# yhz0/SQLP

Measured on AMD Instinct MI355X. Metric: stage-2 subproblems/sec + cut-gen HBM GB/s on STORM, higher is better.
Workload: dtype f64

## Files before the change

### include/twosd_hip.h

```cpp
#ifndef TWOSD_HIP_H
#define TWOSD_HIP_H

#include <stdint.h>

#ifdef __cplusplus
extern "C" {
#endif

typedef struct twosd_ctx twosd_ctx;

enum {
    TWOSD_OK = 0,
    TWOSD_E_ARG = -1,
    TWOSD_E_DEVICE = -2,
    TWOSD_E_STATE = -3,
    TWOSD_E_LP = -4,
    TWOSD_E_UNSUPPORTED = -5
};

enum { TWOSD_LP_OPTIMAL = 0, TWOSD_LP_INFEASIBLE = 1, TWOSD_LP_ITER_LIMIT = 2, TWOSD_LP_NUMERIC = 3 };

const char *twosd_last_error(void);

const char *twosd_version(void);
// ... 152 lines not shown
int twosd_bootstrap_count_of_word(uint32_t u);
int twosd_bootstrap_counts(twosd_ctx *ctx, int M, uint64_t seed, uint64_t first_index, int64_t count, uint8_t *out);

int twosd_bootstrap_counts_vr(twosd_ctx *ctx, int M, uint64_t seed, uint64_t first_index, int64_t count, uint8_t *out,
                              const twosd_sampling *plan);

int twosd_reform_cuts(twosd_ctx *ctx, int epi, int H, const int *handles, int M, uint64_t seed, uint64_t index_offset,
                      double *alpha, double *beta, double *weight_mark, double *total_weight);
int twosd_reform_partial_len(twosd_ctx *ctx, int H, const int *handles, int M, int64_t *n_u64, int64_t *n_f64);
int twosd_reform_partial(twosd_ctx *ctx, int epi, int H, const int *handles, int M, uint64_t seed, uint64_t index_offset,
                         double total_weight, uint64_t *d_u64, double *d_f64);
int twosd_reform_finalize(twosd_ctx *ctx, int H, const int *handles, int M, double total_weight, const uint64_t *d_u64,
                          const double *d_f64, double *alpha, double *beta, double *weight_mark, double *total_weight_out);
int twosd_reform_cuts_vr(twosd_ctx *ctx, int epi, int H, const int *handles, int M, uint64_t seed, uint64_t index_offset,
                         double *alpha, double *beta, double *weight_mark, double *total_weight, const twosd_sampling *plan);
int twosd_reform_partial_vr(twosd_ctx *ctx, int epi, int H, const int *handles, int M, uint64_t seed, uint64_t index_offset,
                            double total_weight, uint64_t *d_u64, double *d_f64, const twosd_sampling *plan);
int twosd_reform_last_ms(twosd_ctx *ctx, double *ms2);

int twosd_last_timings(twosd_ctx *ctx, double *us5);

int twosd_last_lp_stats(twosd_ctx *ctx, int64_t *pivots_sum, int *pivots_max);
int twosd_last_lp_eta_entries(twosd_ctx *ctx, int64_t *entries, int64_t *retries);

int twosd_last_objective(twosd_ctx *ctx, double *weighted_sum, double *weight_sum);

int twosd_last_lp_iters(twosd_ctx *ctx, int N, int *iters, int *status);

int twosd_set_refresh_kcap(twosd_ctx *ctx, int kcap);

int twosd_last_lp_ops(twosd_ctx *ctx, int64_t *row_ops, int *row_width);

int twosd_debug_stamps(twosd_ctx *ctx, uint64_t *out10, int reset);

#ifdef __cplusplus
}
#endif
#endif
```

### sqlp_amd/_lib.py

```python
from __future__ import annotations

import ctypes as C
import os

_HERE = os.path.dirname(os.path.abspath(__file__))
LIB_PATH = os.path.join(_HERE, f"libtwosd_hip_{os.environ['TWOSD_LIB']}.so" if os.environ.get("TWOSD_LIB")
                        else "libtwosd_hip.so")

TWOSD_OK = 0
ERRORS = {-1: "TWOSD_E_ARG", -2: "TWOSD_E_DEVICE", -3: "TWOSD_E_STATE", -4: "TWOSD_E_LP",
          -5: "TWOSD_E_UNSUPPORTED"}
LP_OPTIMAL, LP_INFEASIBLE, LP_ITER_LIMIT, LP_NUMERIC = 0, 1, 2, 3

P = C.c_void_p
I = C.c_int
D = C.c_double
SIGNATURES = [
    ("twosd_last_error", C.c_char_p, []),
    ("twosd_version", C.c_char_p, []),
    ("twosd_create", I, [I, P]),
    ("twosd_destroy", I, [P]),
    ("twosd_set_template", I, [P, I, I, I, P, P, P, P, P, P, P, P, P, P, P, I]),
    ("twosd_lp_shape", I, [P, P, P, P]),
    ("twosd_canonical_form", I, [I, I, P, P, P, P, P, P, P, P, I, P, P, P, P, P, P, P, P, P, P, P, P, P, P, P]),
# ... 20 lines not shown
    ("twosd_moments_merge", I, [P, P, P]),
    ("twosd_moments_of_values", I, [P, C.c_int64, P, P, P]),
    ("twosd_evaluate_moments", I, [P, P, C.c_int64, C.c_int64, C.c_uint64, P]),
    ("twosd_evaluate_paired", I, [P, P, P, C.c_int64, C.c_int64, C.c_uint64, P, P, P]),
    ("twosd_evaluate_ci", I, [P, P, C.c_uint64, C.c_int64, C.c_int64, C.c_int64, D, D, D, D, P, P, P]),
    ("twosd_solve_batch", I, [P, I, P, I, I, P, P, P, P]),
    ("twosd_solve_values", I, [P, P, I, P, P, P, P, P]),
    ("twosd_dvs_push", I, [P, I, P, P, P]),
    ("twosd_dvs_size", I, [P, P]),
    ("twosd_dvs_get", I, [P, I, I, P]),
    ("twosd_dvs_clear", I, [P]),
    ("twosd_dvs_truncate", I, [P, I]),
    ("twosd_dvs_fingerprint", I, [P, P]),
    ("twosd_solve_push", I, [P, I, P, I, I, P, P, P]),
    ("twosd_last_push_reps", I, [P, P]),
    ("twosd_last_push_mode", I, [P, P]),
    ("twosd_build_cut", I, [P, I, P, D, P, P, P, P, P]),
    ("twosd_cut_partial_len", I, [P, P, P]),
    ("twosd_cut_partial", I, [P, I, P, D, D, P, P, P, P]),
    ("twosd_cut_finalize", I, [P, P, P, P, P, P]),
    ("twosd_last_timings", I, [P, P]),
    ("twosd_last_lp_stats", I, [P, P, P]),
    ("twosd_last_lp_eta_entries", I, [P, P, P]),
    ("twosd_last_lp_ops", I, [P, P, P]),
    ("twosd_debug_stamps", I, [P, P, I]),
    ("twosd_last_lp_iters", I, [P, I, P, P]),
    ("twosd_set_refresh_kcap", I, [P, I]),
    ("twosd_refresh_train", I, [P, I, P, I, I, P, P, P]),
    ("twosd_refresh_train_ex", I, [P, I, P, I, I, I, P, P, P, P]),
    ("twosd_refresh_cap_stats", I, [P, P, P]),
    ("twosd_training_cap", I, [P, C.c_int64, C.c_int64, P]),
    ("twosd_cut_stats", I, [P, P]),
    ("twosd_cut_pass", I, [P, P, P]),
    ("twosd_cut_pass_kind", I, [P, P, P, P]),
    ("twosd_cut_debug_scores", I, [P, I, P, P, C.c_int64, P, P]),
    ("twosd_select_refresh_bases", I, [P, P, P, P, I, I, P, P, P]),
    ("twosd_last_objective", I, [P, P, P]),
    ("twosd_refresh_train_bases", I, [P, P, P, P]),
    ("twosd_refresh_build_local", I, [P, I, P, P]),
    ("twosd_refresh_pack", I, [P, P]),
    ("twosd_refresh_assemble", I, [P, I, P, C.c_int64, I, P, P, P, P]),
    ("twosd_pool_candidate_picks", I, [P, I, P, I, I, I, P, P]),
    ("twosd_pool_set_candidates", I, [P, I, I, I, P, P]),
    ("twosd_picks_keep", I, [P, I, P]),
    ("twosd_picks_info", I, [P, I, P, P, P]),
    ("twosd_picks_get", I, [P, I, P]),
# ... 65 lines not shown
```

### sqlp_amd/csrc/lp_batch.hip

```cpp
#include <hip/hip_runtime.h>
#include <algorithm>
#include <cmath>
#include <cstdio>
#include <cstdlib>
#include <vector>
#include "twosd_internal.h"
#include "twosd_ctx.h"

using namespace twosd;

int twosd::run_lp(twosd_ctx *c, const double *x, const double *d_dv, int N, const LpRun &o) {
    const bool want_pi = o.want_pi, want_y = o.want_y;
    const bool list = o.d_list != nullptr;
    const int NL = list ? o.nlist : N;
    int rc;
    if ((rc = prepare_x(c, x))) return rc;
    if (list && c->pool.size() > 1 && (size_t)N > c->d_pool_pick.cap) return fail(TWOSD_E_STATE, "LP list mode: no recorded pool picks");
    const int m = c->L.m, n = c->L.n, MP = c->MP, R = c->R;
    if (N > c->out_cap) {
        size_t cap = std::max<size_t>(N, 1024);
        if ((rc = c->d_obj.alloc(cap)) || (rc = c->d_status.alloc(cap)) || (rc = c->d_iters.alloc(cap)) ||
            (rc = c->d_ops.alloc(cap)) || (rc = c->d_etan.alloc(cap)))
            return rc;
        c->d_pi.release(); c->d_y.release();
        c->out_cap = (int)cap;
    }
    if (want_pi && (size_t)NL * m > c->d_pi.cap && (rc = c->d_pi.alloc((size_t)c->out_cap * m))) return rc;
    if (o.want_key && (size_t)N > c->d_vkey.cap && (rc = c->d_vkey.alloc((size_t)c->out_cap))) return rc;
    if (o.want_bkey && (size_t)N > c->d_bkey.cap && (rc = c->d_bkey.alloc((size_t)c->out_cap))) return rc;
    if (want_y && (size_t)N * n > c->d_y.cap && (rc = c->d_y.alloc((size_t)c->out_cap * n))) return rc;
    if (!c->d_queue && (rc = c->d_queue.alloc((size_t)kMaxQueueGroups * kQueueStride))) return rc;
    {
        const int CH = c->CH;
        int kmax = c->kmax_override > 0 ? c->kmax_override : std::min(256, std::max(64, 2 * m + 32));
        if (c->kmax_override <= 0 && 2 * m + 32 > kmax) {
            const int b0 = hyper_max_blocks_per_cu(R, CH, kmax, c->k);
            for (int k2 = std::min(1024, (2 * m + 32) & ~31); k2 > kmax; k2 -= 32)
                if (hyper_max_blocks_per_cu(R, CH, k2, c->k) >= b0) { kmax = k2; break; }
        }
        const int ecap = (int)std::min<long long>(INT32_MAX / 2, (long long)std::max(4096, 32 * MP) * std::max(256, kmax) / 256);
        int bpc = hyper_max_blocks_per_cu(R, CH, kmax, c->k);
        if (const char *e = getenv("TWOSD_BPC")) bpc = std::min(bpc, std::max(1, atoi(e)));
        if (bpc < 1)
            return fail(TWOSD_E_UNSUPPORTED, "LP kernel: LDS slice too large (m2 = %d, n2 = %d; LP: %d rows, %d columns; k = %d)",
                        c->m2_user, c->n2_user, m, n, c->k);
        const int nblocks = std::max(1, std::min((NL + kWavesPerBlock - 1) / kWavesPerBlock, bpc * c->num_cus));
        const size_t slots = (size_t)nblocks * kWavesPerBlock;
        if (slots > c->earena_slots || ecap != c->earena_cap) {
            if ((rc = c->d_eidx.alloc(slots * ecap)) || (rc = c->d_evals.alloc(slots * ecap))) return rc;
            c->earena_slots = slots;
            c->earena_cap = ecap;
        }
        HIPCHK(hipMemsetAsync(c->d_queue, 0, sizeof(int) * kMaxQueueGroups * kQueueStride, c->stream));
        HyperParams H{};
        H.m = m; H.n = n; H.k = c->k; H.N = NL; H.kmax = kmax; H.ecap = ecap;
        H.kcap = o.kcap > 0 ? std::min(o.kcap, kmax) : kmax;
        H.retry = o.kcap > 0 ? 0 : 1;
        H.colptr = c->d_colptr; H.rowidx = c->d_rowidx; H.val = c->d_val; H.q = c->d_q; H.btype = c->d_btype;
        H.wcp = c->d_wcp; H.wcc = c->d_wcc; H.wcv = c->d_wcv;
        H.bcp = c->d_bcp; H.bci = c->d_bci; H.bcv = c->d_bcv;
        H.brptr = c->d_brptr; H.brcol = c->d_brcol; H.brval = c->d_brval;
        H.kslot = c->d_kslot; H.kix = c->d_kix; H.kv = c->d_kv; H.kcoef = c->d_kcoef;
        H.xbase = c->d_xbase; H.d0 = c->d_d0; H.hb0 = c->d_hb0;
        H.basic0 = c->d_basic0; H.fixedmask = c->d_fixedmask; H.ubmask = c->d_ubmask;
        H.dv = d_dv; H.eidx = c->d_eidx; H.evals = c->d_evals; H.queue = c->d_queue;
        H.qgroups = std::max(1, std::min(16, nblocks));
        if (const char *e = getenv("TWOSD_QGROUPS")) H.qgroups = std::max(1, std::min({kMaxQueueGroups, nblocks, atoi(e)}));
        H.obj = c->d_obj; H.pi = want_pi ? c->d_pi : nullptr; H.y = want_y ? c->d_y : nullptr;
        H.vkey = o.want_key ? c->d_vkey : nullptr;
        H.key_zero = 1e-12;
        if (const char *e = getenv("TWOSD_KEY_ZERO")) H.key_zero = atof(e);
        H.bkey = o.want_bkey ? c->d_bkey : nullptr;
        if (o.want_etas) {
            const size_t need = list ? (size_t)NL : (size_t)N;
            if (need * 4096 > (size_t)INT32_MAX)
                return fail(TWOSD_E_UNSUPPORTED, "eta files of %zu solves exceed the 2^31-entry arena (at most %d)", need,
                            INT32_MAX / 4096);
            const size_t cap_need = std::max(std::max<size_t>(need, 256) * 4096, c->eo_min_cap);
// ... 43 lines not shown
                int w = 0;
                for (int t = 0; t < R; ++t) w = std::max(w, ks[(size_t)p * (R + 1) + t + 1] - ks[(size_t)p * (R + 1) + t]);
                ws[p] = w;
                mean += w;
            }
            std::sort(ws.begin(), ws.end());
            fprintf(stderr, "LP start: ELL width w over %d bases: min %d, median %d, mean %.2f, p90 %d, max %d\n", H.npool, ws.front(),
                    ws[ws.size() / 2], mean / H.npool, ws[ws.size() * 9 / 10], ws.back());
        }
        HIPCHK(hipEventRecord(c->ev[EV_LP_BEGIN], c->stream));
        const int *order = nullptr;
        if (list) {
            order = o.d_list;
        } else if (H.npool > 1) {
            if ((rc = select_pool(c, d_dv, N, c->d_pool_pick, 0))) return rc;
            order = c->d_order;
        }
        HIPCHK(hipEventRecord(c->ev[EV_LP_SELECTED], c->stream));
        if (order || H.npool > 1) {
            if ((rc = c->d_qrec.fit(std::max<size_t>(NL, 1024)))) return rc;
            HIPCHK(launch_queue_records(order, H.npool > 1 ? c->d_pool_pick : nullptr, c->d_qrec, NL, c->stream));
            H.qrec = c->d_qrec;
        }
        HIPCHK(launch_hyper(R, CH, H, nblocks, hyper_lds_bytes(R, CH, kmax, c->k), c->stream));
        HIPCHK(hipEventRecord(c->ev[EV_LP_END], c->stream));
        HIPCHK(hipStreamSynchronize(c->stream));
        float ms = 0, ms_sel = 0;
        hipEventElapsedTime(&ms, c->ev[EV_LP_SELECTED], c->ev[EV_LP_END]);
        hipEventElapsedTime(&ms_sel, c->ev[EV_LP_BEGIN], c->ev[EV_LP_SELECTED]);
        if (list) {
            if (o.lp_us_out) *o.lp_us_out = 1e3 * ms;
            return TWOSD_OK;
        }
        c->last.N = N;
        c->last.lp_us = 1e3 * ms;
        c->last.sel_us = 1e3 * ms_sel;
        return TWOSD_OK;
    }
}

__global__ void __launch_bounds__(256) lp_stats_kernel(int N, const int *__restrict__ its, const long long *__restrict__ ops,
                                                      const int *__restrict__ st, const int *__restrict__ etan,
                                                      unsigned long long *out) {
    __shared__ unsigned long long red[4][5];
    unsigned long long a = 0, b = 0, d = 0, e = 0;
    unsigned long long mx = 0;
    for (int s = blockIdx.x * blockDim.x + threadIdx.x; s < N; s += gridDim.x * blockDim.x) {
// ... 184 lines not shown
    us5[T_POOL_SELECT] = c->last.sel_us;
    return TWOSD_OK;
}

extern "C" int twosd_last_lp_eta_entries(twosd_ctx *c, int64_t *entries, int64_t *retries) {
    if (!c || !entries) return fail(TWOSD_E_ARG, "last_lp_eta_entries: NULL");
    *entries = c->last.eta_entries;
    if (retries) *retries = c->last.retries;
    return TWOSD_OK;
}

extern "C" int twosd_last_lp_stats(twosd_ctx *c, int64_t *sum, int *mx) {
    if (!c) return fail(TWOSD_E_ARG, "last_lp_stats: NULL");
    if (sum) *sum = c->last.pivots_sum;
    if (mx) *mx = c->last.pivots_max;
    return TWOSD_OK;
}

extern "C" int twosd_last_lp_iters(twosd_ctx *c, int N, int *iters, int *status) {
    if (!c || N < 0 || N > c->out_cap || !c->d_iters) return fail(TWOSD_E_ARG, "last_lp_iters: N = %d outside the last batch", N);
    HIPCHK(hipStreamSynchronize(c->stream));
    if (iters) HIPCHK(hipMemcpy(iters, c->d_iters, sizeof(int) * N, hipMemcpyDeviceToHost));
    if (status) HIPCHK(hipMemcpy(status, c->d_status, sizeof(int) * N, hipMemcpyDeviceToHost));
    return TWOSD_OK;
}

extern "C" int twosd_debug_stamps(twosd_ctx *c, uint64_t *out10, int reset) {
    if (!c || !out10) return fail(TWOSD_E_ARG, "debug_stamps: NULL");
    for (int i = 0; i < 10; ++i) out10[i] = 0;
    if (!c->d_stamps) return TWOSD_OK;
    HIPCHK(hipMemcpy(out10, c->d_stamps, sizeof(uint64_t) * 10, hipMemcpyDeviceToHost));
    if (reset) HIPCHK(hipMemset(c->d_stamps, 0, sizeof(uint64_t) * 16));
    return TWOSD_OK;
}

extern "C" int twosd_last_lp_ops(twosd_ctx *c, int64_t *row_ops, int *row_width) {
    if (!c) return fail(TWOSD_E_ARG, "last_lp_ops: NULL");
    if (row_ops) *row_ops = c->last.ops_sum;
    if (row_width) *row_width = 1;
    return TWOSD_OK;
}

__global__ void gather_rows_kernel(int U, int m, const int *__restrict__ list, const double *__restrict__ pi, double *__restrict__ out) {
    const size_t tot = (size_t)U * m;
    for (size_t i = (size_t)blockIdx.x * blockDim.x + threadIdx.x; i < tot; i += (size_t)gridDim.x * blockDim.x) {
        const int u = (int)(i / m), r = (int)(i % m);
// ... 98 lines not shown
```

### sqlp_amd/csrc/lp_hyper.hip

```cpp
#include <hip/hip_runtime.h>
#include <math.h>
#include <type_traits>
#include "twosd_internal.h"
#include "wave_ops.h"

namespace twosd {

#define HTOL_P 1e-9
#define HTOL_D 1e-9
#define HTOL_PIV 1e-9
#define HPI_ZERO 1e-12


#ifdef TWOSD_STAMPS
#define STAMP_DECL unsigned long long st_acc[10] = {0, 0, 0, 0, 0, 0, 0, 0, 0, 0}; \
    unsigned long long st_last = __builtin_amdgcn_s_memtime();
#define STAMP(i)                                                      \
    {                                                                 \
        const unsigned long long t_ = __builtin_amdgcn_s_memtime();   \
        st_acc[i] += t_ - st_last;                                    \
        st_last = t_;                                                 \
    }
#define STAMP_FLUSH                                                                         \
    if (lane == 0 && P.stamps)                                                              \
// ... 104 lines not shown
    int v = 0;
    H_SLOT_SWITCH(__builtin_amdgcn_readfirstlane(p >> 6), R, {
        int u = a[SL];
        asm volatile("" : "+v"(u));
        v = __builtin_amdgcn_readlane(u, p & 63);
    })
    return v;
}

__device__ __forceinline__ int h_prefix_count(uint64_t m) {
    return __builtin_amdgcn_mbcnt_hi((unsigned)(m >> 32), __builtin_amdgcn_mbcnt_lo((unsigned)m, 0u));
}

__device__ __forceinline__ const __attribute__((address_space(4))) HyperParams *h_args() {
    uint64_t a = (uint64_t)__builtin_amdgcn_kernarg_segment_ptr();
    asm volatile("" : "+s"(a));
    return (const __attribute__((address_space(4))) HyperParams *)a;
}
#define CP (*h_args())

static __host__ __device__ inline int hyper_union_doubles(int R, int C) {
    return 128 * R > 64 * C ? 128 * R : 64 * C;
}
static __host__ __device__ inline size_t hyper_slice_bytes(int R, int C, int kmax, int k) {
    const int kmaxp = (kmax + 3) & ~3;
    return 8 * (size_t)hyper_union_doubles(R, C) + 8 * (size_t)((k + 1) & ~1) + 8 * 64 + 4 * 64 + 4 * 64 + 2 * kmaxp +
           4 * (kmaxp + 4);
}
size_t hyper_lds_bytes(int R, int C, int kmax, int k) { return (size_t)kWavesPerBlock * hyper_slice_bytes(R, C, kmax, k); }

#ifndef TWOSD_ETA_G
#define TWOSD_ETA_G 2
#endif
constexpr int EG = TWOSD_ETA_G;
#ifndef TWOSD_REC_UNROLL
#define TWOSD_REC_UNROLL 1
#endif
#ifndef TWOSD_XB_U
#define TWOSD_XB_U 1
#endif
constexpr int XU = TWOSD_XB_U;
#ifndef TWOSD_HYPER_WPE
#define TWOSD_HYPER_WPE(R) ((R) >= 9 ? 2 : 3)
#endif

template <int R, int C, bool FULL>
__global__ void __launch_bounds__(256, TWOSD_HYPER_WPE(R)) lp_hyper_kernel(HyperParams P) {
    extern __shared__ double lds_raw[];
    using Mask = typename std::conditional<(C > 32), uint64_t, uint32_t>::type;
    const int lane = threadIdx.x & 63;
    const int wid = threadIdx.x >> 6;
    constexpr int MP = 64 * R;
    constexpr int UD = 128 * R > 64 * C ? 128 * R : 64 * C;
    const int kmaxp = (P.kmax + 3) & ~3;
    const int ncol = P.n + P.m;
    char *slice = reinterpret_cast<char *>(lds_raw) + (size_t)wid * hyper_slice_bytes(R, C, P.kmax, P.k);
    double *ut = reinterpret_cast<double *>(slice);
    double *rho = ut + MP;
    double *alpha = ut;
    double *dvl = ut + UD;
    double *lstv = dvl + ((P.k + 1) & ~1);
    int *lsti = reinterpret_cast<int *>(lstv + 64);
    int *smark = lsti + 64;
    unsigned short *etap = reinterpret_cast<unsigned short *>(smark + 64);
    int *etaoff = reinterpret_cast<int *>(etap + kmaxp);

    const int m = P.m, n = P.n;
    const int slot_id = blockIdx.x * kWavesPerBlock + wid;
    int *eidx = P.eidx + (size_t)slot_id * P.ecap;
    double *evals = P.evals + (size_t)slot_id * P.ecap;
    const uint64_t fixedm = CP.fixedmask[lane];
    const uint64_t ubm = CP.ubmask[lane];

    for (int j = lane; j < UD; j += 64) ut[j] = 0.0;
    smark[lane] = 0;
    h_wave_sync();
    STAMP_DECL

    const int G = CP.qgroups;
    const int g0 = blockIdx.x % G;
    int gt = 0;
    int q_lo = 0, q_hi = 0;
    auto group_of = [&](int gi) { return g0 + gi < G ? g0 + gi : g0 + gi - G; };
    auto range_set = [&]() {
        const int g = group_of(gt);
        q_lo = (int)(((long long)P.N * g) / G);
        q_hi = (int)(((long long)P.N * (g + 1)) / G);
    };
    auto claim_issue = [&]() -> int {
        int t = 0;
        if (lane == 0 && gt < G) t = atomicAdd(CP.queue + group_of(gt) * kQueueStride, 1);
        return t;
    };
// ... 106 lines not shown
#pragma unroll
                for (int uu = 0; uu < XU; ++uu)
#pragma unroll
                    for (int t = 0; t < R; ++t) {
                        const double v = fma(kvv[uu][t], dg[uu][t], xB[t]);
                        xB[t] = u0 + uu < len[t] ? v : xB[t];
                    }
            }
            uint64_t ub = ubm;
            asm volatile("" : "+v"(ub));
#pragma unroll
            for (int c = 0; c < C; ++c) d[c] = h_flip(d0r[c], ((ub >> c) & 1) << 63);
            if (attempt == 0 && q_nx >= 0) {
                s_nx = has_rec ? __builtin_amdgcn_readfirstlane(rcn.x) : q_nx;
                pb_nx = has_rec ? __builtin_amdgcn_readfirstlane(rcn.y) : 0;
            }
        }
        K = 0; status = TWOSD_LP_OPTIMAL; eoff = 0;
        if (lane == 0) etaoff[0] = 0;
        h_wave_sync();
        STAMP(0)

        auto eta_group = [&](int t0, int dir, int (&gi)[EG], double (&gv)[EG], int (&gn)[EG], int (&go)[EG]) {
#pragma unroll
            for (int g = 0; g < EG; ++g) {
                const int tt = t0 + dir * g;
                const bool ok = (tt >= 0) & (tt < K);
                const int tc = ok ? tt : 0;
                const int o0 = etaoff[tc], o1 = etaoff[tc + 1];
                go[g] = ok ? o0 : 0;
                gn[g] = ok ? o1 - o0 : 0;
                const bool mine = lane < gn[g];
                const int at = mine ? go[g] + lane : 0;
                const int ix = eidx[at];
                const double vx = evals[at];
                gi[g] = mine ? ix : 0;
                gv[g] = mine ? vx : 0.0;
            }
        };
        for (;;) {
            double bnum = 0.0, bden = 1.0, bdel = 0.0;
            int br = 0x7fffffff;
#pragma unroll
            for (int t = 0; t < R; ++t) {
                const int bt = hb[t] & 3;
                const bool inf = (hb[t] >= 0) & (((xB[t] < -HTOL_P) & (bt != BT_G)) | ((xB[t] > HTOL_P) & ((bt & 1) != 0)));
                if (__builtin_amdgcn_ballot_w64(inf) != 0 && inf) {
                    const double dl = xB[t];
                    const double num = dl * dl, den = (double)wd[t];
                    if (num * bden > bnum * den) { bnum = num; bden = den; br = 64 * t + lane; bdel = dl; }
                }
            }
            const ArgBest1 lr = warg_max1(bnum / bden, br, bdel);
            const int r = lr.idx;
            STAMP(1)
            if (lr.key == 0.0) break;
            if (K >= P.kcap) { status = TWOSD_LP_ITER_LIMIT; break; }
            const double delta = lr.p0;

            auto price_batch = [&](int nb) {
                h_wave_sync();
                int p0 = 0, len = 0;
// ... 27 lines not shown
                    lstv[pos] = gr;
                }
                nops += rlen;
                if (nzm != 0) price_batch(__popcll(nzm));
            } else {
                {
                    double one = 1.0;
                    asm volatile("" : "+v"(one));
                    if (lane == (r & 63)) ut[r] = one;
                }
                h_wave_sync();
                const int gp0 = lane <= K ? (lane == 0 ? r : (int)etap[K - lane]) : -1;
                int bp0 = 0, bp1 = 0;
                if (gp0 >= 0) {
                    bp0 = brptr[gp0];
                    bp1 = brptr[gp0 + 1];
                }
                {
                    auto apply = [&](int tg, const int (&gi)[EG], const double (&gv)[EG], const int (&gn)[EG], const int (&go)[EG]) {
#pragma unroll
                        for (int g = 0; g < EG; ++g) {
                            const int tt = tg - g;
                            if (tt < 0) break;
                            const double ug = gv[g] != 0.0 ? ut[gi[g]] : 0.0;
                            if (gn[g] <= 64 && __builtin_amdgcn_ballot_w64(ug != 0.0) == 0) {
                                nops += gn[g];
                                continue;
                            }
                            double acc = ug * gv[g];
                            for (int e = 64 + lane; e < gn[g]; e += 64) acc = fma(ut[eidx[go[g] + e]], evals[go[g] + e], acc);
                            acc = wsum(acc);
                            nops += gn[g];
                            if (lane == 0) ut[etap[tt]] = acc;
                            h_wave_sync();
                        }
                    };
                    int ai[EG], an[EG], ao[EG], bi[EG], bn[EG], bo[EG];
                    double av[EG], bv[EG];
                    if (K <= 2 * EG) {
                        for (int tg = K - 1; tg >= 0; tg -= EG) {
                            eta_group(tg, -1, ai, av, an, ao);
                            apply(tg, ai, av, an, ao);
                        }
                    } else {
                        eta_group(K - 1, -1, ai, av, an, ao);
                        for (int tg = K - 1; tg >= 0;) {
                            eta_group(tg - EG, -1, bi, bv, bn, bo);
                            apply(tg, ai, av, an, ao);
                            tg -= EG;
                            if (tg < 0) break;
                            eta_group(tg - EG, -1, ai, av, an, ao);
                            apply(tg, bi, bv, bn, bo);
                            tg -= EG;
// ... 67 lines not shown
                const bool el = (((cand >> c) & 1) != 0) & (a > HTOL_PIV);
                snz = h_uniform(snz | ((Mask)(__builtin_amdgcn_ballot_w64(av != 0.0) != 0) << c));
                if (__builtin_amdgcn_ballot_w64(el) != 0) {
                    sel |= (Mask)1 << c;
                    const double nu = d[c] + HTOL_D;
                    const bool better = el & (nu * bde < bnu * a);
                    bnu = better ? nu : bnu;
                    bde = better ? a : bde;
                    elm |= (Mask)el << c;
                }
                __builtin_amdgcn_sched_barrier(0);
            }
            const double thmax = wmin(bnu / bde);
            if (thmax == INFINITY) {
                status = TWOSD_LP_INFEASIBLE;
                h_wave_sync();
#pragma unroll
                for (int c = 0; c < C; ++c) alpha[64 * c + lane] = 0.0;
                break;
            }
            double bA = 0.0, bD = 0.0;
            int bq = 0x7fffffff;
            apf = alpha[lane];
#pragma unroll
            for (int c = 0; c < C; ++c) {
                const double av = apf;
                if (c + 1 < C) apf = alpha[64 * (c + 1) + lane];
                if ((sel >> c) & 1) {
                    const double a = h_flip(av, sgm);
                    const bool ok = (((elm >> c) & 1) != 0) & (d[c] <= thmax * a) & (a > bA);
                    bA = ok ? a : bA;
                    bD = ok ? d[c] : bD;
                    bq = ok ? 64 * c + lane : bq;
                }
                __builtin_amdgcn_sched_barrier(0);
            }
            const ArgBest1 eq = warg_max1(bA, bq, bD);
            const int q = eq.idx;
            STAMP(5)
            if (eq.key == 0.0) {
                status = TWOSD_LP_NUMERIC;
                h_wave_sync();
#pragma unroll
                for (int c = 0; c < C; ++c) alpha[64 * c + lane] = 0.0;
                break;
            }
            const double thetaD = eq.p0 / eq.key;
            int fq = q;
            asm volatile("" : "+v"(fq));
            const bool fcol = q < n;
            int fn0 = 0, fn1 = 1, fcc = 0, fp0 = 0, fp1 = 0;
            double ffa = 0.0;
            apf = alpha[lane];
#pragma unroll
            for (int c = 0; c < C; ++c) {
                if (c == 0 && fcol) {
// ... 29 lines not shown
                    if (pw < np1) {
                        const int cc = P.rowidx[pw];
                        fa = P.val[pw];
                        p0 = bcp[cc];
                        len = bcp[cc + 1] - p0;
                    }
                    nops += h_seg_scatter(p0, len, fa, P.bci, P.bcv, ut, smark, lane);
                }
            }
            h_wave_sync();
            {
                auto apply = [&](int tg, const int (&gi)[EG], const double (&gv)[EG], const int (&gn)[EG], const int (&go)[EG]) {
#pragma unroll
                    for (int g = 0; g < EG; ++g) {
                        const int tt = tg + g;
                        if (tt >= K) break;
                        const int p = etap[tt];
                        const double vp = ut[p];
                        if (vp != 0.0) {
                            if (lane < gn[g]) {
                                if (gi[g] == p) ut[p] = gv[g] * vp;
                                else lds_add(&ut[gi[g]], gv[g] * vp);
                            }
                            for (int e = 64 + lane; e < gn[g]; e += 64) {
                                const int i = eidx[go[g] + e];
                                const double ev = evals[go[g] + e];
                                if (i == p) ut[p] = ev * vp;
                                else lds_add(&ut[i], ev * vp);
                            }
                            nops += gn[g];
                            h_wave_sync();
                        }
                    }
                };
                int ai[EG], an[EG], ao[EG], bi[EG], bn[EG], bo[EG];
                double av[EG], bv[EG];
                if (K <= 2 * EG) {
                    for (int tg = 0; tg < K; tg += EG) {
                        eta_group(tg, 1, ai, av, an, ao);
                        apply(tg, ai, av, an, ao);
                    }
                } else {
                    eta_group(0, 1, ai, av, an, ao);
                    for (int tg = 0; tg < K;) {
                        eta_group(tg + EG, 1, bi, bv, bn, bo);
                        apply(tg, ai, av, an, ao);
                        tg += EG;
                        if (tg >= K) break;
                        eta_group(tg + EG, 1, ai, av, an, ao);
                        apply(tg, bi, bv, bn, bo);
                        tg += EG;
// ... 3 lines not shown
            const double arq = ut[r];
            double col[R];
#pragma unroll
            for (int t = 0; t < R; ++t) col[t] = ut[64 * t + lane];
            h_wave_sync();
#pragma unroll
            for (int t = 0; t < R; ++t) ut[64 * t + lane] = 0.0;
            STAMP(7)
            if (fabs(arq) < 1e-12) { status = TWOSD_LP_NUMERIC; h_wave_sync(); break; }

            const double thetaP = delta / arq;
            const double inv_arq = 1.0 / arq;
            float wrr = 0.0f;
            H_SLOT_SWITCH(__builtin_amdgcn_readfirstlane(r >> 6), R, {
                int u = __builtin_bit_cast(int, wd[SL]);
                asm volatile("" : "+v"(u));
                wrr = __builtin_bit_cast(float, __builtin_amdgcn_readlane(u, r & 63));
            })
            int cnt = 0;
#pragma unroll
            for (int t = 0; t < R; ++t) cnt += __popcll(__ballot(col[t] != 0.0));
            if (eoff + cnt > P.ecap) { status = TWOSD_LP_ITER_LIMIT; h_wave_sync(); break; }
            int base = eoff;
#pragma unroll
            for (int t = 0; t < R; ++t) {
                const int i = 64 * t + lane;
                const bool nz = col[t] != 0.0;
                const bool isr = i == r;
                const uint64_t bal = __ballot(nz);
                const double ratio = col[t] * inv_arq;
                if (nz) {
                    const int pos = base + h_prefix_count(bal);
                    eidx[pos] = i;
                    evals[pos] = isr ? inv_arq : -ratio;
                }
                const float nw = (float)((double)wrr * inv_arq * inv_arq);
                const float cand = (float)(ratio * ratio * (double)wrr);
                const double xo = fma(-thetaP, col[t], xB[t]);
                xB[t] = isr ? thetaP : (nz ? xo : xB[t]);
                wd[t] = isr ? (nw > 1.0f ? nw : 1.0f) : ((nz & (cand > wd[t])) ? cand : wd[t]);
                base += __popcll(bal);
            }
            eoff += cnt;
            if (lane == 0) {
                etap[K] = (unsigned short)r;
                etaoff[K + 1] = eoff;
            }
            ++K;
            const int lh = h_get_row_i<R>(hb, r);
            const int leaving = lh >> 2;
            {
                const int ls = __builtin_amdgcn_readfirstlane(leaving >> 6), qs = __builtin_amdgcn_readfirstlane(q >> 6);
                const double dlv = (delta > 0) == ((lh & 3) == BT_G) ? thetaD : -thetaD;
                const bool lme = lane == (leaving & 63), qme = lane == (q & 63);
                H_SLOT_SWITCH(ls, C, {
                    double v = lme ? dlv : d[SL];
                    asm volatile("" : "+v"(v));
                    d[SL] = v;
                })
                H_SLOT_SWITCH(qs, C, {
                    double v = qme ? 0.0 : d[SL];
                    asm volatile("" : "+v"(v));
                    d[SL] = v;
                })
                if (lme) bmask &= ~(1ull << ls);
                if (qme) bmask |= 1ull << qs;
                {
                    const int nh = q * 4 + (int)P.btype[q];
                    const bool rme = lane == (r & 63);
                    H_SLOT_SWITCH(__builtin_amdgcn_readfirstlane(r >> 6), R, {
                        int v = rme ? nh : hb[SL];
                        asm volatile("" : "+v"(v));
                        hb[SL] = v;
                    })
                }
            }
            ++it;
            h_wave_sync();
            STAMP(8)
        }
        if (status == TWOSD_LP_OPTIMAL || pb == 0 || !CP.retry) break;
        if (lane == 0 && CP.retries) atomicAdd(CP.retries, 1ull);
        pb = 0;
        }
        double dvn0 = 0.0, dvn1 = 0.0, kcn0 = 0.0, kcn1 = 0.0;
        int ksn = 0, t_claim = 0;
        if (q_nx >= 0) {
            const auto *A = h_args();
            t_claim = claim_issue();
            if (lane <= R) ksn = A->kslot[pb_nx * (R + 1) + lane];
            if (dv_pf) {
                const double *dvs = A->dv + (size_t)s_nx * P.k;
                if (lane < P.k) { dvn0 = dvs[lane]; kcn0 = A->kcoef[lane]; }
                if (lane + 64 < P.k) { dvn1 = dvs[lane + 64]; kcn1 = A->kcoef[lane + 64]; }
            }
        }

        double objv = NAN;
        unsigned long long keyv = 0;
        if (status == TWOSD_LP_OPTIMAL) {
            const double *qc = CP.q;
            double qv[R];
#pragma unroll
// ... 43 lines not shown
                        const double v = fabs(dc) <= zt ? 0.0 : dc;
                        const unsigned long long b = ((unsigned long long)__double_as_longlong(v) + (1ull << 28)) >> 29;
                        h += mix64(((unsigned long long)(j - n) << 35) | b);
                    }
                }
#pragma unroll
                for (int o = 32; o > 0; o >>= 1) h += __shfl_xor(h, o);
                keyv = h;
            }
        }
        if constexpr (FULL) {
        if (status == TWOSD_LP_OPTIMAL && (P.pi || P.y)) {
            const double *qc = CP.q;
#pragma unroll
            for (int t = 0; t < R; ++t) {
                const int j = hb[t] >> 2;
                const bool bq = hb[t] >= 0 && j < n;
                const double qj = qc[bq ? j : 0];
                ut[64 * t + lane] = bq ? qj : 0.0;
            }
            h_wave_sync();
            for (int tt = K - 1; tt >= 0; --tt) {
                const int off = etaoff[tt], nnz = etaoff[tt + 1] - off;
                double acc = 0.0;
                for (int e = lane; e < nnz; e += 64) acc = fma(ut[eidx[off + e]], evals[off + e], acc);
                acc = wsum(acc);
                nops += nnz;
                if (lane == 0) ut[etap[tt]] = acc;
                h_wave_sync();
            }
            double pv[R];
            double pmax = 0.0;
#pragma unroll
            for (int t = 0; t < R; ++t) {
                const int cc = 64 * t + lane;
                const int e0 = cc < m ? bcp[cc] : 0, e1 = cc < m ? bcp[cc + 1] : 0;
                double a = 0.0;
#pragma unroll TWOSD_REC_UNROLL
                for (int e = e0; e < e1; ++e) a = fma(ut[P.bci[e]], P.bcv[e], a);
                pv[t] = a;
                pmax = fmax(pmax, fabs(a));
            }
            nops += P.bnnz[pb];
            pmax = wmax(pmax);
            const double zt = HPI_ZERO * (1.0 + pmax);
#pragma unroll
            for (int t = 0; t < R; ++t)
                if (fabs(pv[t]) <= zt) pv[t] = 0.0;
// ... 26 lines not shown
        if (P.head_out) {
            const size_t ho = (size_t)(P.pi_by_pos ? qpos : s) * m;
#pragma unroll
            for (int t = 0; t < R; ++t)
                if (64 * t + lane < m) P.head_out[ho + 64 * t + lane] = hb[t] >> 2;
        }
        if (P.bkey && status == TWOSD_LP_OPTIMAL) {
            unsigned long long h = 0;
#pragma unroll
            for (int t = 0; t < R; ++t)
                if (64 * t + lane < m) h += mix64((unsigned long long)(hb[t] >> 2));
#pragma unroll
            for (int o = 32; o > 0; o >>= 1) h += __shfl_xor(h, o);
            if (lane == 0) P.bkey[s] = h;
        }
        if (P.eo_K) {
            const int erow = P.pi_by_pos ? qpos : s;
            unsigned long long off64 = 0;
            if (lane == 0 && status == TWOSD_LP_OPTIMAL) off64 = atomicAdd(P.eo_used, (unsigned long long)eoff);
            off64 = __shfl(off64, 0);
            const bool ok = status == TWOSD_LP_OPTIMAL && off64 + (unsigned long long)eoff <= (unsigned long long)P.eo_cap;
            const int off = ok ? (int)off64 : 0;
            if (ok) {
                for (int e = lane; e < eoff; e += 64) {
                    P.eo_eidx[off + e] = eidx[e];
                    P.eo_evals[off + e] = evals[e];
                }
                for (int t = lane; t < K; t += 64) P.eo_etap[(size_t)erow * P.kmax + t] = etap[t];
                for (int t = lane; t <= K; t += 64) P.eo_etaoff[(size_t)erow * (P.kmax + 1) + t] = etaoff[t];
            }
            if (lane == 0) {
                P.eo_K[erow] = ok ? K : -1;
                P.eo_off[erow] = off;
                P.eo_pb[erow] = pb;
            }
        }
        }
        {
            const auto *A = h_args();
            double *const o_obj = A->obj;
            int *const o_status = A->status, *const o_iters = A->iters, *const o_etan = A->etan, *const o_pick = A->pool_pick;
            long long *const o_ops = A->ops;
            unsigned long long *const o_key = A->vkey;
            const int su = __builtin_amdgcn_readfirstlane(s);
            if (lane == 0) {
                o_obj[su] = objv;
                o_status[su] = status;
                o_iters[su] = it;
                if (o_ops) o_ops[su] = (long long)nops;
// ... 322 lines not shown
    switch (C) {                                    \
        case 2: return FN<R, 2>(__VA_ARGS__);       \
        case 4: return FN<R, 4>(__VA_ARGS__);       \
        case 8: return FN<R, 8>(__VA_ARGS__);       \
        case 14: return FN<R, 14>(__VA_ARGS__);     \
        case 16: return FN<R, 16>(__VA_ARGS__);     \
        case 28: return FN<R, 28>(__VA_ARGS__);     \
        case 32: return FN<R, 32>(__VA_ARGS__);     \
        case 64: return FN<R, 64>(__VA_ARGS__);     \
    }
#endif

hipError_t launch_hyper(int R, int C, const HyperParams &p, int nblocks, size_t lds, hipStream_t s) {
    switch (R) {
        case 1: HYPER_C_SWITCH(1, hl, p, nblocks, lds, s); break;
        case 2: HYPER_C_SWITCH(2, hl, p, nblocks, lds, s); break;
        case 4: HYPER_C_SWITCH(4, hl, p, nblocks, lds, s); break;
        case 9: HYPER_C_SWITCH(9, hl, p, nblocks, lds, s); break;
        case 16: HYPER_C_SWITCH(16, hl, p, nblocks, lds, s); break;
    }
    return hipErrorInvalidValue;
}

int hyper_max_blocks_per_cu(int R, int C, int kmax, int k) {
    const size_t lds = hyper_lds_bytes(R, C, kmax, k);
    if (lds > 160 * 1024) return 0;
    switch (R) {
        case 1: HYPER_C_SWITCH(1, ho, lds); break;
        case 2: HYPER_C_SWITCH(2, ho, lds); break;
        case 4: HYPER_C_SWITCH(4, ho, lds); break;
        case 9: HYPER_C_SWITCH(9, ho, lds); break;
        case 16: HYPER_C_SWITCH(16, ho, lds); break;
    }
    return 1;
}

}
```

### sqlp_amd/csrc/twosd_internal.h

```cpp
#pragma once
#include <hip/hip_runtime.h>
#include <stdint.h>
#include <string>
#include <vector>
#include "twosd_hip.h"
#include "devbuf.h"

namespace twosd {

constexpr int kWave = 64;
constexpr int kWavesPerBlock = 4;
constexpr int kMaxColsPerLane = 64;

enum : int { BT_Y = 0, BT_G = 1, BT_L = 2, BT_E = 3 };


constexpr int kQueueStride = 32;
constexpr int kMaxQueueGroups = 64;
struct HyperParams {
    int m, n, k, N, kmax, ecap;
    int kcap;
    int retry;
    const int *colptr, *rowidx; const double *val;
    const double *q; const int8_t *btype;
    const int *wcp, *wcc; const double *wcv;
    const int *bcp, *bci; const double *bcv;
    const int *brptr, *brcol; const double *brval;
    const int *kslot, *kix; const double *kv;
    const double *kcoef;
    const double *xbase;
    const double *d0;
    const int *hb0;
    const uint64_t *basic0, *fixedmask, *ubmask;
    const double *dv;
    int *eidx; double *evals;
    int *queue;
    int qgroups;
    double *obj;
    int *status, *iters;
    long long *ops;
    int *etan;
    int *pool_pick;
    unsigned long long *vkey;
    double *pi, *y;
    unsigned long long *retries;
// ... 82 lines not shown
    int *pick;
    float cw;
    float *key;
    float *pkey; int *ppick;
};
struct PoolRefineParams {
    int N, k, ncand;
    const double *dv, *kcoef;
    const float *cinf;
    const int *sptr, *send;
    const int2 *rec;
    const int *order, *cand;
    int *pick;
    const float *key;
    float cw;
    float *pkey; int *pci;
};
hipError_t launch_pool_refine(const PoolRefineParams &p, hipStream_t s);
size_t pool_select_lds_bytes(int k);
int pool_select_split(int N, int npool);
int pool_refine_split(int N, int ncand);
hipError_t sort_by_pool(const int *pick, int *order, int N, int npool, void *tmp, size_t *tmp_bytes, hipStream_t s);
hipError_t launch_pool_select(const PoolSelParams &p, hipStream_t s);
size_t hyper_lds_bytes(int R, int C, int kmax, int k);
int hyper_rows_per_lane(int m);
int hyper_cols_per_lane(int ncols);
hipError_t launch_hyper(int R, int C, const HyperParams &p, int nblocks, size_t lds, hipStream_t s);
hipError_t launch_queue_records(const int *order, const int *pick, int2 *qrec, int N, hipStream_t s);
int hyper_max_blocks_per_cu(int R, int C, int kmax, int k);


struct SampleParams {
    int N, k;
    unsigned long long seed, first_index;
    const int *kind;
    const int *off;
    const double *val, *prob;
    const double *p0, *p1;
    const double *tmpl;
    double *out;
};
hipError_t launch_sample(const SampleParams &S, hipStream_t st);
hipError_t launch_sample_plan(const SampleParams &S, int mode, int G, hipStream_t st);

struct HostLP {
    int m = 0, n = 0;
    std::vector<int> colptr, rowidx;
    std::vector<double> val, q;
    std::vector<char> sense;
};
bool dense_inverse(int m, const std::vector<double> &A, std::vector<double> &Ainv);
void basis_matrix(const HostLP &L, const std::vector<int> &head, std::vector<double> &B);
// ... 23 lines not shown
```

Measured before the change: 18.32 million.

## Keep leading eta-file entries in LDS when occupancy allows

Adds a per-wave LDS region for the first EL eta-file entries (16-bit row index plus f64 value). FTRAN/BTRAN, pivot updates and the eta export read from LDS when an eta group lies fully inside that region, and fall back to global memory otherwise. EL is picked by a binary search that keeps blocks-per-CU unchanged, then kmax is grown under the same constraint. The goal is to cut global/HBM traffic on short eta files, at the cost of extra branching and possible interaction with occupancy. The change also adds sizing and debug query APIs and moves the iteration-count update out of the loop.

New measurement: 17.55 million. 4.2% lower.

```diff
diff --git a/include/twosd_hip.h b/include/twosd_hip.h
--- a/include/twosd_hip.h
+++ b/include/twosd_hip.h
@@ -198,6 +198,9 @@
 
 int twosd_last_lp_stats(twosd_ctx *ctx, int64_t *pivots_sum, int *pivots_max);
 int twosd_last_lp_eta_entries(twosd_ctx *ctx, int64_t *entries, int64_t *retries);
+int twosd_last_lp_detail(twosd_ctx *ctx, int N, int *etan, uint64_t *vkey);
+int twosd_lp_sizing(twosd_ctx *ctx, int *out4);
+int twosd_lp_sizing_model(int m, int ncols, int k, int el_req, int reg_blocks, int *out4);
 
 int twosd_last_objective(twosd_ctx *ctx, double *weighted_sum, double *weight_sum);
 
diff --git a/sqlp_amd/_lib.py b/sqlp_amd/_lib.py
--- a/sqlp_amd/_lib.py
+++ b/sqlp_amd/_lib.py
@@ -66,6 +66,9 @@
     ("twosd_last_timings", I, [P, P]),
     ("twosd_last_lp_stats", I, [P, P, P]),
     ("twosd_last_lp_eta_entries", I, [P, P, P]),
+    ("twosd_last_lp_detail", I, [P, I, P, P]),
+    ("twosd_lp_sizing", I, [P, P]),
+    ("twosd_lp_sizing_model", I, [I, I, I, I, I, P]),
     ("twosd_last_lp_ops", I, [P, P, P]),
     ("twosd_debug_stamps", I, [P, P, I]),
     ("twosd_last_lp_iters", I, [P, I, P, P]),
diff --git a/sqlp_amd/csrc/lp_batch.hip b/sqlp_amd/csrc/lp_batch.hip
--- a/sqlp_amd/csrc/lp_batch.hip
+++ b/sqlp_amd/csrc/lp_batch.hip
@@ -8,6 +8,33 @@
 #include "twosd_ctx.h"
 
 using namespace twosd;
+
+static HyperSizing lp_sizing(const twosd_ctx *c) {
+    int el_req = -1;
+    if (const char *e = getenv("TWOSD_ETA_LDS")) el_req = std::max(0, atoi(e));
+    const int R = c->R, CH = c->CH, k = c->k;
+    return hyper_sizing(c->L.m, c->kmax_override, el_req, [=](int kmax, int el) { return hyper_max_blocks_per_cu(R, CH, kmax, k, el); });
+}
+
+extern "C" int twosd_lp_sizing(twosd_ctx *c, int *out4) {
+    if (!c || !out4 || !c->has_template) return fail(TWOSD_E_ARG, "lp_sizing: NULL or no template");
+    HIPCHK(hipSetDevice(c->device));
+    const HyperSizing z = lp_sizing(c);
+    out4[0] = z.kmax; out4[1] = z.el; out4[2] = z.bpc;
+    out4[3] = (int)hyper_lds_bytes(c->R, c->CH, z.kmax, c->k, z.el);
+    return TWOSD_OK;
+}
+
+extern "C" int twosd_lp_sizing_model(int m, int ncols, int k, int el_req, int reg_blocks, int *out4) {
+    const int R = hyper_rows_per_lane(m), CH = hyper_cols_per_lane(ncols);
+    if (R < 0 || CH < 0 || k < 0 || reg_blocks < 1 || !out4) return fail(TWOSD_E_ARG, "lp_sizing_model: bad arguments");
+    const HyperSizing z = hyper_sizing(m, 0, el_req, [=](int kmax, int el) {
+        return (int)std::min<size_t>((size_t)reg_blocks, (size_t)160 * 1024 / hyper_lds_bytes(R, CH, kmax, k, el));
+    });
+    out4[0] = z.kmax; out4[1] = z.el; out4[2] = z.bpc;
+    out4[3] = (int)hyper_lds_bytes(R, CH, z.kmax, k, z.el);
+    return TWOSD_OK;
+}
 
 int twosd::run_lp(twosd_ctx *c, const double *x, const double *d_dv, int N, const LpRun &o) {
     const bool want_pi = o.want_pi, want_y = o.want_y;
@@ -32,14 +59,10 @@
     if (!c->d_queue && (rc = c->d_queue.alloc((size_t)kMaxQueueGroups * kQueueStride))) return rc;
     {
         const int CH = c->CH;
-        int kmax = c->kmax_override > 0 ? c->kmax_override : std::min(256, std::max(64, 2 * m + 32));
-        if (c->kmax_override <= 0 && 2 * m + 32 > kmax) {
-            const int b0 = hyper_max_blocks_per_cu(R, CH, kmax, c->k);
-            for (int k2 = std::min(1024, (2 * m + 32) & ~31); k2 > kmax; k2 -= 32)
-                if (hyper_max_blocks_per_cu(R, CH, k2, c->k) >= b0) { kmax = k2; break; }
-        }
+        const HyperSizing sz = lp_sizing(c);
+        const int kmax = sz.kmax, el = sz.el;
         const int ecap = (int)std::min<long long>(INT32_MAX / 2, (long long)std::max(4096, 32 * MP) * std::max(256, kmax) / 256);
-        int bpc = hyper_max_blocks_per_cu(R, CH, kmax, c->k);
+        int bpc = hyper_max_blocks_per_cu(R, CH, kmax, c->k, el);
         if (const char *e = getenv("TWOSD_BPC")) bpc = std::min(bpc, std::max(1, atoi(e)));
         if (bpc < 1)
             return fail(TWOSD_E_UNSUPPORTED, "LP kernel: LDS slice too large (m2 = %d, n2 = %d; LP: %d rows, %d columns; k = %d)",
@@ -53,7 +76,7 @@
         }
         HIPCHK(hipMemsetAsync(c->d_queue, 0, sizeof(int) * kMaxQueueGroups * kQueueStride, c->stream));
         HyperParams H{};
-        H.m = m; H.n = n; H.k = c->k; H.N = NL; H.kmax = kmax; H.ecap = ecap;
+        H.m = m; H.n = n; H.k = c->k; H.N = NL; H.kmax = kmax; H.ecap = ecap; H.el = el;
         H.kcap = o.kcap > 0 ? std::min(o.kcap, kmax) : kmax;
         H.retry = o.kcap > 0 ? 0 : 1;
         H.colptr = c->d_colptr; H.rowidx = c->d_rowidx; H.val = c->d_val; H.q = c->d_q; H.btype = c->d_btype;
@@ -143,7 +166,7 @@
             HIPCHK(launch_queue_records(order, H.npool > 1 ? c->d_pool_pick : nullptr, c->d_qrec, NL, c->stream));
             H.qrec = c->d_qrec;
         }
-        HIPCHK(launch_hyper(R, CH, H, nblocks, hyper_lds_bytes(R, CH, kmax, c->k), c->stream));
+        HIPCHK(launch_hyper(R, CH, H, nblocks, hyper_lds_bytes(R, CH, kmax, c->k, el), c->stream));
         HIPCHK(hipEventRecord(c->ev[EV_LP_END], c->stream));
         HIPCHK(hipStreamSynchronize(c->stream));
         float ms = 0, ms_sel = 0;
@@ -374,6 +397,15 @@
     HIPCHK(hipStreamSynchronize(c->stream));
     if (iters) HIPCHK(hipMemcpy(iters, c->d_iters, sizeof(int) * N, hipMemcpyDeviceToHost));
     if (status) HIPCHK(hipMemcpy(status, c->d_status, sizeof(int) * N, hipMemcpyDeviceToHost));
+    return TWOSD_OK;
+}
+
+extern "C" int twosd_last_lp_detail(twosd_ctx *c, int N, int *etan, uint64_t *vkey) {
+    if (!c || N < 0 || N > c->out_cap || !c->d_etan) return fail(TWOSD_E_ARG, "last_lp_detail: N = %d outside the last batch", N);
+    if (vkey && (size_t)N > c->d_vkey.cap) return fail(TWOSD_E_STATE, "last_lp_detail: the last batch computed no dual keys");
+    HIPCHK(hipStreamSynchronize(c->stream));
+    if (etan) HIPCHK(hipMemcpy(etan, c->d_etan, sizeof(int) * N, hipMemcpyDeviceToHost));
+    if (vkey) HIPCHK(hipMemcpy(vkey, c->d_vkey, sizeof(uint64_t) * N, hipMemcpyDeviceToHost));
     return TWOSD_OK;
 }
 
diff --git a/sqlp_amd/csrc/lp_hyper.hip b/sqlp_amd/csrc/lp_hyper.hip
--- a/sqlp_amd/csrc/lp_hyper.hip
+++ b/sqlp_amd/csrc/lp_hyper.hip
@@ -150,12 +150,14 @@
 static __host__ __device__ inline int hyper_union_doubles(int R, int C) {
     return 128 * R > 64 * C ? 128 * R : 64 * C;
 }
-static __host__ __device__ inline size_t hyper_slice_bytes(int R, int C, int kmax, int k) {
+static __host__ __device__ inline size_t hyper_slice_bytes(int R, int C, int kmax, int k, int el) {
     const int kmaxp = (kmax + 3) & ~3;
     return 8 * (size_t)hyper_union_doubles(R, C) + 8 * (size_t)((k + 1) & ~1) + 8 * 64 + 4 * 64 + 4 * 64 + 2 * kmaxp +
-           4 * (kmaxp + 4);
-}
-size_t hyper_lds_bytes(int R, int C, int kmax, int k) { return (size_t)kWavesPerBlock * hyper_slice_bytes(R, C, kmax, k); }
+           4 * (kmaxp + 4) + 10 * (size_t)el;
+}
+size_t hyper_lds_bytes(int R, int C, int kmax, int k, int el) {
+    return (size_t)kWavesPerBlock * hyper_slice_bytes(R, C, kmax, k, el);
+}
 
 #ifndef TWOSD_ETA_G
 #define TWOSD_ETA_G 2
@@ -182,7 +184,8 @@
     constexpr int UD = 128 * R > 64 * C ? 128 * R : 64 * C;
     const int kmaxp = (P.kmax + 3) & ~3;
     const int ncol = P.n + P.m;
-    char *slice = reinterpret_cast<char *>(lds_raw) + (size_t)wid * hyper_slice_bytes(R, C, P.kmax, P.k);
+    const int EL = P.el;
+    char *slice = reinterpret_cast<char *>(lds_raw) + (size_t)wid * hyper_slice_bytes(R, C, P.kmax, P.k, EL);
     double *ut = reinterpret_cast<double *>(slice);
     double *rho = ut + MP;
     double *alpha = ut;
@@ -190,13 +193,25 @@
     double *lstv = dvl + ((P.k + 1) & ~1);
     int *lsti = reinterpret_cast<int *>(lstv + 64);
     int *smark = lsti + 64;
-    unsigned short *etap = reinterpret_cast<unsigned short *>(smark + 64);
+    double *elv = reinterpret_cast<double *>(smark + 64);
+    unsigned short *eli = reinterpret_cast<unsigned short *>(elv + EL);
+    unsigned short *etap = eli + EL;
     int *etaoff = reinterpret_cast<int *>(etap + kmaxp);
 
     const int m = P.m, n = P.n;
     const int slot_id = blockIdx.x * kWavesPerBlock + wid;
     int *eidx = P.eidx + (size_t)slot_id * P.ecap;
     double *evals = P.evals + (size_t)slot_id * P.ecap;
+    auto eta_resident = [&](int end) -> bool { return __builtin_amdgcn_readfirstlane(end) <= EL; };
+    auto eta_entry = [&](bool res, int at, int &ix, double &vx) {
+        if (res) {
+            ix = eli[at];
+            vx = elv[at];
+        } else {
+            ix = eidx[at];
+            vx = evals[at];
+        }
+    };
     const uint64_t fixedm = CP.fixedmask[lane];
     const uint64_t ubm = CP.ubmask[lane];
 
@@ -349,6 +364,26 @@
         STAMP(0)
 
         auto eta_group = [&](int t0, int dir, int (&gi)[EG], double (&gv)[EG], int (&gn)[EG], int (&go)[EG]) {
+            int tl = dir > 0 ? t0 : t0 - (EG - 1);
+            tl = tl < 0 ? 0 : (tl >= K ? K - 1 : tl);
+            if (!eta_resident(etaoff[tl + 1])) {
+#pragma unroll
+                for (int g = 0; g < EG; ++g) {
+                    const int tt = t0 + dir * g;
+                    const bool ok = (tt >= 0) & (tt < K);
+                    const int tc = ok ? tt : 0;
+                    const int o0 = etaoff[tc], o1 = etaoff[tc + 1];
+                    go[g] = ok ? o0 : 0;
+                    gn[g] = ok ? o1 - o0 : 0;
+                    const bool mine = lane < gn[g];
+                    const int at = mine ? go[g] + lane : 0;
+                    const int ix = eidx[at];
+                    const double vx = evals[at];
+                    gi[g] = mine ? ix : 0;
+                    gv[g] = mine ? vx : 0.0;
+                }
+                return;
+            }
 #pragma unroll
             for (int g = 0; g < EG; ++g) {
                 const int tt = t0 + dir * g;
@@ -358,13 +393,23 @@
                 go[g] = ok ? o0 : 0;
                 gn[g] = ok ? o1 - o0 : 0;
                 const bool mine = lane < gn[g];
-                const int at = mine ? go[g] + lane : 0;
-                const int ix = eidx[at];
-                const double vx = evals[at];
-                gi[g] = mine ? ix : 0;
-                gv[g] = mine ? vx : 0.0;
+                int ix = 0;
+                double vx = 0.0;
+                if (eta_resident(o1)) {
+                    if (mine) {
+                        ix = eli[go[g] + lane];
+                        vx = elv[go[g] + lane];
+                    }
+                } else {
+                    const int at = mine ? go[g] + lane : 0;
+                    ix = eidx[at];
+                    vx = evals[at];
+                }
+                gi[g] = ix;
+                gv[g] = vx;
             }
         };
+        auto group_resident = [&](int o, int len) -> bool { return eta_resident(o + len); };
         for (;;) {
             double bnum = 0.0, bden = 1.0, bdel = 0.0;
             int br = 0x7fffffff;
@@ -438,13 +483,23 @@
                         for (int g = 0; g < EG; ++g) {
                             const int tt = tg - g;
                             if (tt < 0) break;
-                            const double ug = gv[g] != 0.0 ? ut[gi[g]] : 0.0;
+                            const bool mine = lane < gn[g];
+                            const double ev0 = mine ? gv[g] : 0.0;
+                            const double ug = ev0 != 0.0 ? ut[mine ? gi[g] : 0] : 0.0;
                             if (gn[g] <= 64 && __builtin_amdgcn_ballot_w64(ug != 0.0) == 0) {
                                 nops += gn[g];
                                 continue;
                             }
-                            double acc = ug * gv[g];
-                            for (int e = 64 + lane; e < gn[g]; e += 64) acc = fma(ut[eidx[go[g] + e]], evals[go[g] + e], acc);
+                            double acc = ug * ev0;
+                            if (gn[g] > 64) {
+                                const bool res = group_resident(go[g], gn[g]);
+                                for (int e = 64 + lane; e < gn[g]; e += 64) {
+                                    int i;
+                                    double ev;
+                                    eta_entry(res, go[g] + e, i, ev);
+                                    acc = fma(ut[i], ev, acc);
+                                }
+                            }
                             acc = wsum(acc);
                             nops += gn[g];
                             if (lane == 0) ut[etap[tt]] = acc;
@@ -558,6 +613,8 @@
             double bA = 0.0, bD = 0.0;
             int bq = 0x7fffffff;
             apf = alpha[lane];
+            int lq = lane;
+            asm volatile("" : "+v"(lq));
 #pragma unroll
             for (int c = 0; c < C; ++c) {
                 const double av = apf;
@@ -567,7 +624,7 @@
                     const bool ok = (((elm >> c) & 1) != 0) & (d[c] <= thmax * a) & (a > bA);
                     bA = ok ? a : bA;
                     bD = ok ? d[c] : bD;
-                    bq = ok ? 64 * c + lane : bq;
+                    bq = ok ? 64 * c + lq : bq;
                 }
                 __builtin_amdgcn_sched_barrier(0);
             }
@@ -643,11 +700,15 @@
                                 if (gi[g] == p) ut[p] = gv[g] * vp;
                                 else lds_add(&ut[gi[g]], gv[g] * vp);
                             }
-                            for (int e = 64 + lane; e < gn[g]; e += 64) {
-                                const int i = eidx[go[g] + e];
-                                const double ev = evals[go[g] + e];
-                                if (i == p) ut[p] = ev * vp;
-                                else lds_add(&ut[i], ev * vp);
+                            if (gn[g] > 64) {
+                                const bool res = group_resident(go[g], gn[g]);
+                                for (int e = 64 + lane; e < gn[g]; e += 64) {
+                                    int i;
+                                    double ev;
+                                    eta_entry(res, go[g] + e, i, ev);
+                                    if (i == p) ut[p] = ev * vp;
+                                    else lds_add(&ut[i], ev * vp);
+                                }
                             }
                             nops += gn[g];
                             h_wave_sync();
@@ -697,6 +758,7 @@
             for (int t = 0; t < R; ++t) cnt += __popcll(__ballot(col[t] != 0.0));
             if (eoff + cnt > P.ecap) { status = TWOSD_LP_ITER_LIMIT; h_wave_sync(); break; }
             int base = eoff;
+            const bool eres = eoff + cnt <= EL;
 #pragma unroll
             for (int t = 0; t < R; ++t) {
                 const int i = 64 * t + lane;
@@ -706,8 +768,14 @@
                 const double ratio = col[t] * inv_arq;
                 if (nz) {
                     const int pos = base + h_prefix_count(bal);
-                    eidx[pos] = i;
-                    evals[pos] = isr ? inv_arq : -ratio;
+                    const double ev = isr ? inv_arq : -ratio;
+                    if (eres) {
+                        eli[pos] = (unsigned short)i;
+                        elv[pos] = ev;
+                    } else {
+                        eidx[pos] = i;
+                        evals[pos] = ev;
+                    }
                 }
                 const float nw = (float)((double)wrr * inv_arq * inv_arq);
                 const float cand = (float)(ratio * ratio * (double)wrr);
@@ -750,10 +818,10 @@
                     })
                 }
             }
-            ++it;
             h_wave_sync();
             STAMP(8)
         }
+        it += K;
         if (status == TWOSD_LP_OPTIMAL || pb == 0 || !CP.retry) break;
         if (lane == 0 && CP.retries) atomicAdd(CP.retries, 1ull);
         pb = 0;
@@ -843,8 +911,14 @@
             h_wave_sync();
             for (int tt = K - 1; tt >= 0; --tt) {
                 const int off = etaoff[tt], nnz = etaoff[tt + 1] - off;
+                const bool res = eta_resident(off + nnz);
                 double acc = 0.0;
-                for (int e = lane; e < nnz; e += 64) acc = fma(ut[eidx[off + e]], evals[off + e], acc);
+                for (int e = lane; e < nnz; e += 64) {
+                    int i;
+                    double ev;
+                    eta_entry(res, off + e, i, ev);
+                    acc = fma(ut[i], ev, acc);
+                }
                 acc = wsum(acc);
                 nops += nnz;
                 if (lane == 0) ut[etap[tt]] = acc;
@@ -917,9 +991,18 @@
             const bool ok = status == TWOSD_LP_OPTIMAL && off64 + (unsigned long long)eoff <= (unsigned long long)P.eo_cap;
             const int off = ok ? (int)off64 : 0;
             if (ok) {
+                int lb = 0;
+                for (int t = lane; t <= K; t += 64) {
+                    const int o = etaoff[t];
+                    lb = o <= EL && o > lb ? o : lb;
+                }
+                lb = __builtin_amdgcn_readlane(h_scan_max(lb), 63);
                 for (int e = lane; e < eoff; e += 64) {
-                    P.eo_eidx[off + e] = eidx[e];
-                    P.eo_evals[off + e] = evals[e];
+                    int i;
+                    double ev;
+                    eta_entry(e < lb, e, i, ev);
+                    P.eo_eidx[off + e] = i;
+                    P.eo_evals[off + e] = ev;
                 }
                 for (int t = lane; t < K; t += 64) P.eo_etap[(size_t)erow * P.kmax + t] = etap[t];
                 for (int t = lane; t <= K; t += 64) P.eo_etaoff[(size_t)erow * (P.kmax + 1) + t] = etaoff[t];
@@ -1288,8 +1371,8 @@
     return hipErrorInvalidValue;
 }
 
-int hyper_max_blocks_per_cu(int R, int C, int kmax, int k) {
-    const size_t lds = hyper_lds_bytes(R, C, kmax, k);
+int hyper_max_blocks_per_cu(int R, int C, int kmax, int k, int el) {
+    const size_t lds = hyper_lds_bytes(R, C, kmax, k, el);
     if (lds > 160 * 1024) return 0;
     switch (R) {
         case 1: HYPER_C_SWITCH(1, ho, lds); break;
diff --git a/sqlp_amd/csrc/twosd_internal.h b/sqlp_amd/csrc/twosd_internal.h
--- a/sqlp_amd/csrc/twosd_internal.h
+++ b/sqlp_amd/csrc/twosd_internal.h
@@ -21,6 +21,7 @@
     int m, n, k, N, kmax, ecap;
     int kcap;
     int retry;
+    int el;
     const int *colptr, *rowidx; const double *val;
     const double *q; const int8_t *btype;
     const int *wcp, *wcc; const double *wcv;
@@ -149,12 +150,32 @@
 int pool_refine_split(int N, int ncand);
 hipError_t sort_by_pool(const int *pick, int *order, int N, int npool, void *tmp, size_t *tmp_bytes, hipStream_t s);
 hipError_t launch_pool_select(const PoolSelParams &p, hipStream_t s);
-size_t hyper_lds_bytes(int R, int C, int kmax, int k);
+size_t hyper_lds_bytes(int R, int C, int kmax, int k, int el);
 int hyper_rows_per_lane(int m);
 int hyper_cols_per_lane(int ncols);
 hipError_t launch_hyper(int R, int C, const HyperParams &p, int nblocks, size_t lds, hipStream_t s);
 hipError_t launch_queue_records(const int *order, const int *pick, int2 *qrec, int N, hipStream_t s);
-int hyper_max_blocks_per_cu(int R, int C, int kmax, int k);
+int hyper_max_blocks_per_cu(int R, int C, int kmax, int k, int el);
+struct HyperSizing { int kmax, el, bpc; };
+template <typename Occ>
+inline HyperSizing hyper_sizing(int m, int kmax_override, int el_req, Occ occ) {
+    constexpr int kEtaLdsTarget = 256;
+    const int base = kmax_override > 0 ? kmax_override : (2 * m + 32 < 64 ? 64 : (2 * m + 32 > 256 ? 256 : 2 * m + 32));
+    HyperSizing z{base, 0, occ(base, 0)};
+    if (z.bpc < 1) return z;
+    int want = (el_req < 0 ? kEtaLdsTarget : el_req) & ~3;
+    if (want > 65532) want = 65532;
+    for (int lo = 0, hi = want; lo < hi;) {
+        const int mid = ((lo + hi) / 2 + 3) & ~3;
+        if (occ(base, mid) >= z.bpc) { lo = mid; z.el = mid; } else { hi = mid - 4; }
+    }
+    if (kmax_override <= 0 && 2 * m + 32 > base) {
+        const int top = (2 * m + 32) & ~31;
+        for (int k2 = top < 1024 ? top : 1024; k2 > base; k2 -= 32)
+            if (occ(k2, z.el) >= z.bpc) { z.kmax = k2; break; }
+    }
+    return z;
+}
 
 
 struct SampleParams {
```
